# skhu101/TDNN-F_NAS

Hardware: AMD Instinct MI355X
Metric: LF-MMI training frames/sec per node (SWBD 7q TDNN-F) (higher is better)
Workload: dtype f32

## Files before the change

tdnn-f_nas_amd/csrc/abi_tdnn.hip:

```cpp
#include <dlfcn.h>
#include <stdlib.h>
#include <string.h>

#include <string>

#include "common.h"
#include "gemm_f32.h"
#include "planes_gemm.h"

namespace tdnnf {

static thread_local std::string g_last_error;

void set_error(const char *fmt, ...) {
  char buf[1024];
  va_list ap;
  va_start(ap, fmt);
  vsnprintf(buf, sizeof(buf), fmt, ap);
  va_end(ap);
  g_last_error = buf;
}
int hip_status(hipError_t e, const char *what) {
  set_error("HIP error %d (%s) in %s", (int)e, hipGetErrorString(e), what);
  return TDNNF_EHIP;
}

Options &options() {
  static Options o;
  return o;
}

namespace {
typedef int (*roctx_push_t)(const char *);
typedef int (*roctx_pop_t)();
roctx_push_t g_roctx_push = nullptr;
roctx_pop_t g_roctx_pop = nullptr;
bool roctx_ready() {
  static const bool ok = [] {
    const char *e = getenv("TDNNF_ROCTX");
    if (e && atoi(e) == 0) return false;
    for (const char *lib : {"librocprofiler-sdk-roctx.so", "librocprofiler-sdk-roctx.so.1", "libroctx64.so", "libroctx64.so.4"}) {
      void *h = dlopen(lib, RTLD_NOW | RTLD_GLOBAL);
      if (!h) continue;
      g_roctx_push = (roctx_push_t)dlsym(h, "roctxRangePushA");
      g_roctx_pop = (roctx_pop_t)dlsym(h, "roctxRangePop");
      if (g_roctx_push && g_roctx_pop) return true;
    }
    return false;
  }();
  return ok;
}
}
TraceRange::TraceRange(const char *name) : on(roctx_ready()) {
  if (on) g_roctx_push(name);
}
TraceRange::~TraceRange() {
  if (on) g_roctx_pop();
}

static bool tdnn_rows_ok(const tdnnf_tdnn_indexes *ix, int rows_in, int N) {
  if (!ix || ix->num_offsets < 1 || ix->num_offsets > TDNNF_MAX_OFFSETS || ix->row_stride < 1) return false;
  for (int i = 0; i < ix->num_offsets; i++) {
    const long long need = (long long)ix->row_offsets[i] + (long long)ix->row_stride * N - (ix->row_stride - 1);
    if (ix->row_offsets[i] < 0 || (N > 0 && rows_in < need)) return false;
  }
  return true;
}

}

using namespace tdnnf;

extern "C" {

const char *tdnnf_last_error(void) { return g_last_error.c_str(); }
int tdnnf_abi_version(void) { return 1; }

static int *option_slot(const char *name) {
  Options &o = options();
  if (!name) return nullptr;
  const struct { const char *n; int *p; } table[] = {{"ng_grouped", &o.ng_grouped}, {"ng_fuse", &o.ng_fuse}, {"ng_early_in", &o.ng_early_in},
                                                     {"wgrad_stream", &o.wgrad_stream}, {"gemm_ring", &o.gemm_ring}, {"planes", &o.planes}, {"den_split", &o.den_split}, {"phase_events", &o.phase_events}, {"wgrad_lag", &o.wgrad_lag}, {"ng_bk", &o.ng_bk}, {"ng_valu", &o.ng_valu}, {"ng_pform", &o.ng_pform}, {"planes_group", &o.planes_group}, {"xent_behind_den", &o.xent_behind_den}, {"ng_early_fork", &o.ng_early_fork}, {"ng_diag_skip", &o.ng_diag_skip}, {"wgrad_small", &o.wgrad_small}, {"splitk_per_cu", &o.splitk_per_cu}, {"gemm_alt_taps", &o.gemm_alt_taps}, {"reverse_passes", &o.reverse_passes}, {"splitk_partial_round", &o.splitk_partial_round}, {"wgrad_on_caller", &o.wgrad_on_caller}, {"den_mw_test_abort", &o.den_mw_test_abort}, {"planes_check_bound", &o.planes_check_bound}};
  for (auto &e : table)
    if (strcmp(e.n, name) == 0) return e.p;
  return nullptr;
}
int tdnnf_set_option(const char *name, int value) {
  int *p = option_slot(name);
  TDNNF_REQUIRE(p, "set_option: unknown option '%s' (ng_grouped, ng_fuse, ng_early_in, wgrad_stream, gemm_ring, planes, den_split)", name ? name : "(null)");
  *p = value;
  return TDNNF_OK;
}
int tdnnf_get_option(const char *name, int *value) {
  int *p = option_slot(name);
  TDNNF_REQUIRE(p && value, "get_option: unknown option '%s'", name ? name : "(null)");
  *value = *p;
  return TDNNF_OK;
}

}

namespace tdnnf {
int tdnn_propagate_impl(const tdnnf_tdnn_indexes *ix, const tdnnf_mat *in, const float *W, int ldw, int Do, int Di,
                        const float *bias, const float *eff_coef, int init_mode, int relu, tdnnf_mat *out, tdnnf_stream stream,
                        float *colstats, int *colstats_rows) {
  TDNNF_REQUIRE(mat_ok(in) && mat_ok(out) && W, "tdnn_propagate: bad matrices");
  TDNNF_REQUIRE(Do > 0 && Di > 0 && in->cols == Di && out->cols == Do, "tdnn_propagate: dims: in.cols=%d Di=%d out.cols=%d Do=%d",
                in ? in->cols : -1, Di, out ? out->cols : -1, Do);
  TDNNF_REQUIRE(tdnn_rows_ok(ix, in->rows, out->rows), "tdnn_propagate: input has too few rows for the time offsets");
  TDNNF_REQUIRE(ldw >= ix->num_offsets * Di, "tdnn_propagate: ldw < K*Di");
  TDNNF_REQUIRE(init_mode >= 0 && init_mode <= 2 && (init_mode != 1 || bias), "tdnn_propagate: init_mode 1 needs a bias");
  RowsGemmArgs a;
  memset(&a, 0, sizeof(a));
  a.A = in->data;
  a.lda = (long long)in->stride * ix->row_stride;
  a.B = W;
  a.ldb = ldw;
  a.C = out->data;
  a.ldc = out->stride;
  a.M = out->rows;
  a.N = Do;
  a.bias = bias;
  a.coef = eff_coef;
  a.init_mode = init_mode;
  a.relu = relu;
  a.colstats = colstats;
  a.colstats_rows = colstats_rows;
  a.nseg = ix->num_offsets;
  for (int i = 0; i < a.nseg; i++) {
    a.seg[i].a_off = (long long)ix->row_offsets[i] * in->stride;
    a.seg[i].b_off = (long long)i * Di;
    a.seg[i].klen = Di;
    a.seg[i].m_lo = 0;
    a.seg[i].m_hi = out->rows;
  }
  TDNNF_HIP(rows_gemm(a, true, (hipStream_t)stream));
  return TDNNF_OK;
}
}

extern "C" {

int tdnnf_tdnn_propagate(const tdnnf_tdnn_indexes *ix, const tdnnf_mat *in, const float *W, int ldw, int Do, int Di,
                         const float *bias, const float *eff_coef, int init_mode, tdnnf_mat *out, tdnnf_stream stream) {
  return tdnn_propagate_impl(ix, in, W, ldw, Do, Di, bias, eff_coef, init_mode, 0, out, stream);
}

}

namespace tdnnf {
int tdnn_backprop_data_impl(const tdnnf_tdnn_indexes *ix, const tdnnf_mat *out_deriv, const float *W, int ldw, int Do,
                            int Di, const float *eff_coef, int overwrite, const tdnnf_mat *add, float add_scale, int add_lo,
                            tdnnf_mat *in_deriv, tdnnf_stream stream) {
  TDNNF_REQUIRE(mat_ok(in_deriv) && mat_ok(out_deriv) && W, "tdnn_backprop_data: bad matrices");
  TDNNF_REQUIRE(Do > 0 && Di > 0 && in_deriv->cols == Di && out_deriv->cols == Do, "tdnn_backprop_data: bad dims");
  TDNNF_REQUIRE(tdnn_rows_ok(ix, in_deriv->rows, out_deriv->rows), "tdnn_backprop_data: in_deriv has too few rows for the time offsets");
  TDNNF_REQUIRE(ldw >= ix->num_offsets * Di, "tdnn_backprop_data: ldw < K*Di");
  const int rho = ix->row_stride, N = out_deriv->rows, K = ix->num_offsets;
  if (N == 0) return TDNNF_OK;
  for (int cls = 0; cls < rho; cls++) {
    RowsGemmArgs a;
    memset(&a, 0, sizeof(a));
    float cf_dummy = 0;
    (void)cf_dummy;
    int nseg = 0, u_max = 0;
// ... 171 lines not shown
```

tdnn-f_nas_amd/csrc/chain.hip:

```cpp
#include <math.h>
#include <string.h>

#include <algorithm>

#include <vector>

#include "common.h"
#include "gemm_f32.h"

struct tdnnf_den_graph {
  int H, A, P;
  struct Sell {
    int nrows, nslices;
    int *base;
    unsigned *row;
    uint2 *arc;
    uint4 *arc4;
    long long entries;
    int mw_max_arcs[9];
  } by_dst, by_src, by_pdf;
  float *init;
  float init_sum;
};

// ... 519 lines not shown
      }
    }
    const float sum = block_sum(local, red, kDenThreads / 64);
    if (gi == 0 && tid == 0) sums[t] = sum;
    if (DIR == 0) {
      for (int h = tid; h < H; h += kDenThreads) {
        const float a = cur[h] + leaky * sum * g.init[h];
        cur[h] = a;
        if (h >= h0 && h < h1) vec[(size_t)t * Hs + h] = a;
      }
    } else {
      const float is = 1.0f / sum;
      for (int h = tid; h < H; h += kDenThreads) {
        const float v = cur[h];
        if (h >= h0 && h < h1) vec[(size_t)t * Hs + h] = v;
        cur[h] = v * is + leaky;
      }
    }
    if (step < T) row_to_x();
    prev_sum = sum;
    __syncthreads();
  }
  if (DIR == 0) {
    float local = 0.f;
    for (int h = tid; h < H; h += kDenThreads) local += cur[h];
    const float tot = block_sum(local, red, kDenThreads / 64);
    if (gi == 0 && tid == 0) {
      logprob[s] = (double)logf(tot) + logcorr;
      sums[T] = tot;
    }
  }
}

__global__ void den_mw_check_kernel(const unsigned *abort_flag, unsigned *host_fallbacks) {
  if (*abort_flag != 0 && threadIdx.x == 0) __hip_atomic_fetch_add(host_fallbacks, 1u, __ATOMIC_RELAXED, __HIP_MEMORY_SCOPE_SYSTEM);
}

constexpr int kGammaThreads = 512;
__global__ __launch_bounds__(kGammaThreads) void den_gamma_kernel(DenDev g, MatView y, int B, int T, float leaky, const float *alpha_all, const float *b_all,
                                                                  const float *S_all, int Hs, float deriv_weight, MatView deriv) {
  extern __shared__ __attribute__((aligned(16))) float smem[];
  __shared__ float red[kGammaThreads / 64];
  const int t = blockIdx.x, s = blockIdx.y, tid = threadIdx.x;
  const int H = g.H, P = g.P, P4 = (P + 3) & ~3, H4 = (H + 3) & ~3;
  float *x = smem, *ad = smem + P4, *bn = ad + H4;
  const float *alpha = alpha_all + ((size_t)s * (T + 1) + t) * Hs;
  const float *bt = b_all + ((size_t)s * (T + 1) + t) * Hs, *bt1 = bt + Hs;
  const float inv = 1.0f / S_all[(size_t)s * (T + 1) + t + 1];
  const float *yr = y.data + (size_t)(t * B + s) * y.stride;
  for (int p = tid; p < P; p += kGammaThreads) x[p] = exp_limited(yr[p]);
  float local = 0.f;
  for (int h = tid; h < H; h += kGammaThreads) {
    const float a = alpha[h];
    ad[h] = a;
    bn[h] = bt1[h] * inv + leaky;
    local += a * bt[h];
  }
  const float Zd = block_sum(local, red, kGammaThreads / 64);
  const float scale = deriv_weight / Zd;
  float *dr = deriv.data + (size_t)(t * B + s) * deriv.stride;
  constexpr int kRows = 12;
  const int nslot = g.by_pdf.nslices * 64, ln = tid & 63;
  auto term = [&](const uint2 a) { return __uint_as_float(a.y) * ad[a.x & 0xffffu] * bn[a.x >> 16]; };
  for (int s0 = tid; s0 < nslot; s0 += kRows * kGammaThreads) {
    int b0[kRows], w[kRows];
    unsigned row[kRows];
#pragma unroll
    for (int k = 0; k < kRows; k++) {
      const int slot = s0 + k * kGammaThreads;
      b0[k] = 0;
      w[k] = 0;
      row[k] = 0xffffffffu;
      if (slot < nslot) {
        b0[k] = g.by_pdf.base[slot >> 6];
        w[k] = (g.by_pdf.base[(slot >> 6) + 1] - b0[k]) >> 6;
        row[k] = g.by_pdf.row[slot];
      }
    }
#pragma unroll
    for (int k = 0; k < kRows; k++) {
      if (row[k] == 0xffffffffu) continue;
      const float acc = sell_row_sum(g.by_pdf.arc + b0[k] + ln, w[k], term);
      dr[row[k]] = scale * acc * x[row[k]];
    }
  }
}
constexpr int kWideBatch = 8;
constexpr int kWideSlices = 2;

struct WideDims {
  int B, NG, SG;
};

typedef unsigned uv4 __attribute__((ext_vector_type(4)));

__global__ __launch_bounds__(256) void den_wide_prep_kernel(MatView y, WideDims d, int P, float *xT) {
  __shared__ float tile[64][65];
  const int t = blockIdx.z, p0 = blockIdx.x * 64, s0 = blockIdx.y * 64, tx = threadIdx.x & 63, ty = threadIdx.x >> 6;
  for (int i = ty; i < 64; i += 4) {
    const int sq = s0 + i, p = p0 + tx;
    tile[i][tx] = (sq < d.B && p < P) ? exp_limited(y.data[(size_t)(t * d.B + sq) * y.stride + p]) : 0.f;
  }
  __syncthreads();
  for (int i = ty; i < 64; i += 4) {
    const int p = p0 + i, sq = s0 + tx;
    if (p < P && sq < d.NG * d.SG) xT[(((size_t)t * d.NG + sq / d.SG) * P + p) * d.SG + sq % d.SG] = tile[tx][i];
  }
}
__global__ __launch_bounds__(256) void den_wide_unprep_kernel(const float *dT, WideDims d, int P, MatView deriv) {
  __shared__ float tile[64][65];
  const int t = blockIdx.z, p0 = blockIdx.x * 64, s0 = blockIdx.y * 64, tx = threadIdx.x & 63, ty = threadIdx.x >> 6;
  for (int i = ty; i < 64; i += 4) {
    const int p = p0 + i, sq = s0 + tx;
    tile[i][tx] = (p < P && sq < d.B) ? dT[(((size_t)t * d.NG + sq / d.SG) * P + p) * d.SG + sq % d.SG] : 0.f;
  }
  __syncthreads();
  for (int i = ty; i < 64; i += 4) {
    const int sq = s0 + i, p = p0 + tx;
    if (sq < d.B && p < P) deriv.data[(size_t)(t * d.B + sq) * deriv.stride + p] = tile[tx][i];
  }
}

__global__ __launch_bounds__(256) void den_wide_init_kernel(DenDev g, WideDims d, int Hs, bool ones, float *v, float *norm) {
  const long long total = (long long)d.NG * Hs * d.SG;
  for (long long e = blockIdx.x * 256LL + threadIdx.x; e < total; e += gridDim.x * 256LL) {
    const int h = (int)((e / d.SG) % Hs);
    v[e] = h < g.H ? (ones ? 1.0f : g.init[h]) : 0.f;
  }
  for (long long e = blockIdx.x * 256LL + threadIdx.x; e < d.B; e += gridDim.x * 256LL) norm[e] = g.init_sum;
}

template <int SG>
struct WideLane {
  static constexpr int RL = 64 / SG;
  static constexpr int IT = 16 / RL;
  int grp, blk, sl, rl, sq, wave, lane;
  bool on;
  __device__ WideLane(const WideDims &d, int g, int b) {
    lane = threadIdx.x & 63;
    wave = threadIdx.x >> 6;
    grp = g;
    blk = b;
    sl = lane % SG;
    rl = lane / SG;
    sq = grp * SG + sl;
    on = sq < d.B;
  }
};
__device__ __forceinline__ int wide_npad(int nblk) { return (nblk + 3) & ~3; }
template <int SG>
__device__ __forceinline__ float wide_norm(const float *part, int nblk, float *norm_out, float *red, const WideLane<SG> &L) {
  constexpr int NQ = 256 / SG;
  const int q = threadIdx.x / SG, nch = wide_npad(nblk) >> 2;
  const float4 *pp = (const float4 *)(part + ((size_t)L.grp * SG + L.sl) * wide_npad(nblk));
  float v = 0.f;
  for (int c0 = q; c0 < nch; c0 += 8 * NQ) {
    float4 f[8];
#pragma unroll
    for (int u = 0; u < 8; u++) f[u] = c0 + u * NQ < nch ? pp[c0 + u * NQ] : make_float4(0.f, 0.f, 0.f, 0.f);
#pragma unroll
    for (int u = 0; u < 8; u++) v += (f[u].x + f[u].y) + (f[u].z + f[u].w);
  }
  red[q * SG + L.sl] = v;
  __syncthreads();
  float tot = 0.f;
#pragma unroll
// ... 698 lines not shown
    hipStream_t st = nullptr;
    hipEvent_t ef = nullptr, ej = nullptr;
  };
  constexpr int kMaxDev = 64;
  static thread_local Set sets[kMaxDev];
  int dev = 0;
  TDNNF_HIP(hipGetDevice(&dev));
  TDNNF_REQUIRE(dev >= 0 && dev < kMaxDev, "chain: device index %d out of range", dev);
  Set &S = sets[dev];
  if (!S.ef) {
    TDNNF_HIP(hipEventCreateWithFlags(&S.ef, hipEventDisableTiming));
    TDNNF_HIP(hipEventCreateWithFlags(&S.ej, hipEventDisableTiming));
  }
  if (aux && !S.st) TDNNF_HIP(hipStreamCreateWithFlags(&S.st, hipStreamNonBlocking));
  if (aux) *aux = S.st;
  *ev_fork = S.ef;
  *ev_join = S.ej;
  return TDNNF_OK;
}

int chain_den(const tdnnf_den_graph *g, const tdnnf_supervision *sp, const tdnnf_mat *y, float leaky, tdnnf_mat *deriv, void *ws,
              hipStream_t s, bool beside_other_work, hipStream_t caller_aux, hipEvent_t ev_recursions, bool *ev_recorded) {
  if (ev_recorded) *ev_recorded = false;
  const int B = sp->B, T = sp->T;
  ChainBufs b = chain_bufs(g, B, T, ws);
  DenDev gd{g->H, g->P, g->by_dst, g->by_src, g->by_pdf, g->init, g->init_sum};
  MatView yv = view(y), dv = view(deriv);
  ProfHbmRange prof(6, (double)B * T * (24.0 * g->A + 12.0 * g->P), s);
  if (b.p.wide) {
    const int Hs = b.p.Hs, P = g->P;
    const WideDims d{B, b.p.NG, b.p.SG};
    const size_t Bw = (size_t)d.NG * d.SG, frame = Bw * Hs, prow = Bw * b.p.wide_blocks;
    const int nsl = kWideSlices;
    auto blocks = [&](const tdnnf_den_graph::Sell &t) { return (t.nslices + nsl - 1) / nsl; };
    const int nb_dst = blocks(g->by_dst), nb_src = blocks(g->by_src);
    float *alphaT = b.alpha, *asum = b.asum, *S = asum + (size_t)(T + 1) * B, *Zd = S + (size_t)(T + 1) * B;
    float *bT = b.gstate, *part = bT + frame * (T + 1), *part2 = part + 2 * prow, *xT = part2 + 2 * prow;
    const dim3 blk(256), tr((P + 63) / 64, (B + 63) / 64, T), ini(grid_for((long long)frame, 256));
    hipStream_t aux_stream;
    hipEvent_t ev_fork, ev_join;
    {
      int rc = den_aux_stream(&aux_stream, &ev_fork, &ev_join);
      if (rc) return rc;
    }
    hipStream_t aux = aux_stream;
    hipLaunchKernelGGL(den_wide_prep_kernel, tr, blk, 0, s, yv, d, P, xT);
    TDNNF_HIP(hipEventRecord(ev_fork, s));
    TDNNF_HIP(hipStreamWaitEvent(aux, ev_fork, 0));
#define WIDE_LAUNCH(kernel, ...)                                      \
  do {                                                                \
    if (d.SG == 16) hipLaunchKernelGGL(kernel<16>, __VA_ARGS__);      \
    else hipLaunchKernelGGL(kernel<32>, __VA_ARGS__);                 \
  } while (0)
    hipLaunchKernelGGL(den_wide_init_kernel, ini, blk, 0, s, gd, d, Hs, false, alphaT, asum);
    for (int t = 1; t <= T; t++)
      WIDE_LAUNCH(den_wide_fwd_kernel, dim3(nb_dst * d.NG), blk, 0, s, gd, d, t, leaky, xT, alphaT, asum, Hs,
                  t > 1 ? part + (size_t)((t - 1) & 1) * prow : (const float *)nullptr, nb_dst, nsl, part + (size_t)(t & 1) * prow);
    WIDE_LAUNCH(den_wide_sum_kernel, dim3(d.NG), blk, 0, s, part + (size_t)(T & 1) * prow, nb_dst, d, asum + (size_t)T * B);
    hipLaunchKernelGGL(den_wide_total_kernel, dim3((B + 255) / 256), blk, 0, s, gd, B, T, leaky, asum, b.den_lp);
    hipLaunchKernelGGL(den_wide_init_kernel, ini, blk, 0, aux, gd, d, Hs, true, bT + (size_t)T * frame, S + (size_t)T * B);
    for (int t = T - 1; t >= 0; t--)
      WIDE_LAUNCH(den_wide_beta_kernel, dim3(nb_src * d.NG), blk, 0, aux, gd, d, t, leaky, xT, bT + (size_t)(t + 1) * frame, S, Hs, bT + (size_t)t * frame,
                  t < T - 1 ? part2 + (size_t)((t + 1) & 1) * prow : (const float *)nullptr, nb_src, nsl, part2 + (size_t)(t & 1) * prow);
    WIDE_LAUNCH(den_wide_sum_kernel, dim3(d.NG), blk, 0, aux, part2, nb_src, d, S);
    TDNNF_HIP(hipEventRecord(ev_join, aux));
    TDNNF_HIP(hipStreamWaitEvent(s, ev_join, 0));
    WIDE_LAUNCH(den_wide_dot_kernel, dim3(T, d.NG), blk, 0, s, gd, d, leaky, alphaT, asum, Hs, bT, Zd);
    WIDE_LAUNCH(den_wide_gamma_kernel, dim3(g->by_pdf.nslices * d.NG, T), blk, 0, s, gd, d, leaky, xT, alphaT, asum, Hs, bT, S, Zd, -sp->weight);
#undef WIDE_LAUNCH
    hipLaunchKernelGGL(den_wide_unprep_kernel, tr, blk, 0, s, xT, d, P, dv);
    TDNNF_LAUNCH_CHECK();
    return TDNNF_OK;
  }
  if (b.p.split && !beside_other_work) {
    const int P4 = (g->P + 3) & ~3, H4 = (g->H + 3) & ~3;
    const size_t lds_beta = sizeof(float) * (P4 + H4), lds_gamma = sizeof(float) * (P4 + 2 * H4);
    float *b_all = b.gstate, *S_all = b_all + (size_t)B * (T + 1) * b.p.Hs;
    hipEvent_t ev_fork, ev_join;
    hipStream_t aux = caller_aux;
    int rc = den_aux_stream(caller_aux ? nullptr : &aux, &ev_fork, &ev_join);
    if (rc) return rc;
    TDNNF_HIP(hipFuncSetAttribute((const void *)den_forward_kernel<true>, hipFuncAttributeMaxDynamicSharedMemorySize, (int)b.p.lds_fwd));
    TDNNF_HIP(hipFuncSetAttribute((const void *)den_beta_kernel<false>, hipFuncAttributeMaxDynamicSharedMemorySize, (int)lds_beta));
    TDNNF_HIP(hipFuncSetAttribute((const void *)den_gamma_kernel, hipFuncAttributeMaxDynamicSharedMemorySize, (int)lds_gamma));
    TDNNF_HIP(hipEventRecord(ev_fork, s));
    TDNNF_HIP(hipStreamWaitEvent(aux, ev_fork, 0));
    int G = mw_groups(g, B, T);
    MwDev *md = mw_dev();
    if (!md) G = 0;
    if (G > 0 && !md->fallbacks) {
      if (hipHostMalloc((void **)&md->fallbacks, sizeof(unsigned), hipHostMallocMapped) != hipSuccess) {
        (void)hipGetLastError();
        md->fallbacks = nullptr;
        G = 0;
      } else {
        *md->fallbacks = 0;
      }
    }
    if (G > 0 && *(volatile unsigned *)md->fallbacks != 0) {
      fprintf(stderr, "tdnnf: the multi-workgroup denominator recursion timed out (its workgroups were not co-resident); the one-workgroup kernels redid the "
                      "minibatch and are used from here on (this device)\n");
      md->off = true;
      G = 0;
    }
    const size_t stage_b = G > 0 ? 256 * (size_t)((std::max(g->by_dst.nslices, g->by_src.nslices) + G - 1) / G) : 0;
    const size_t lds_f = G > 0 ? sizeof(float) * (P4 + H4) + 8 * (size_t)g->by_dst.mw_max_arcs[G] + stage_b : 0;
    const size_t lds_b = G > 0 ? sizeof(float) * (P4 + H4) + 8 * (size_t)g->by_src.mw_max_arcs[G] + stage_b : 0;
    if (G > 0) {
      TDNNF_HIP(hipFuncSetAttribute((const void *)den_mw_kernel<0>, hipFuncAttributeMaxDynamicSharedMemorySize, (int)lds_f));
      TDNNF_HIP(hipFuncSetAttribute((const void *)den_mw_kernel<1>, hipFuncAttributeMaxDynamicSharedMemorySize, (int)lds_b));
      int occ_f = 0, occ_b = 0;
      if (hipOccupancyMaxActiveBlocksPerMultiprocessor(&occ_f, den_mw_kernel<0>, kDenThreads, lds_f) != hipSuccess ||
          hipOccupancyMaxActiveBlocksPerMultiprocessor(&occ_b, den_mw_kernel<1>, kDenThreads, lds_b) != hipSuccess || occ_f < 1 || occ_b < 1 ||
          md->cus <= 0 || 2 * B * G > md->cus) {
        (void)hipGetLastError();
        G = 0;
      }
    }
    if (G > 0) {
      float *mw = S_all + (size_t)B * (T + 1) + 32;
      MwCtl ctl;
      ctl.NSp = (int)mw_slots(g);
      ctl.ctr = reinterpret_cast<unsigned long long *>((reinterpret_cast<uintptr_t>(mw) + 15) & ~(uintptr_t)15);
      ctl.abort_flag = reinterpret_cast<unsigned *>(ctl.ctr + 2 * B);
      ctl.xf = reinterpret_cast<float *>(ctl.ctr + 2 * B + 2);
      ctl.xb = ctl.xf + (size_t)B * 2 * ctl.NSp;
      TDNNF_HIP(hipMemsetAsync(ctl.ctr, 0, sizeof(unsigned long long) * (2 * B + 2), s));
      if (options().den_mw_test_abort) TDNNF_HIP(hipMemsetAsync(ctl.abort_flag, 1, 1, s));
      TDNNF_HIP(hipEventRecord(ev_fork, s));
      TDNNF_HIP(hipStreamWaitEvent(aux, ev_fork, 0));
      hipLaunchKernelGGL(den_mw_kernel<0>, dim3(B * G), dim3(kDenThreads), lds_f, s, gd, ctl, G, yv, B, T, leaky, b.alpha, b.asum, b.p.Hs, b.den_lp);
      hipLaunchKernelGGL(den_mw_kernel<1>, dim3(B * G), dim3(kDenThreads), lds_b, aux, gd, ctl, G, yv, B, T, leaky, b_all, S_all, b.p.Hs, (double *)nullptr);
      hipLaunchKernelGGL(den_forward_kernel<true>, dim3(B), dim3(kDenThreads), b.p.lds_fwd, s, gd, yv, B, T, leaky, b.alpha, b.asum, b.p.Hs, b.den_lp, b.gstate,
                         (const unsigned *)ctl.abort_flag, 0);
      hipLaunchKernelGGL(den_beta_kernel<false>, dim3(B), dim3(kDenThreads), lds_beta, aux, gd, yv, B, T, leaky, b_all, S_all, b.p.Hs, (const unsigned *)ctl.abort_flag, 0);
      hipLaunchKernelGGL(den_mw_check_kernel, dim3(1), dim3(64), 0, s, (const unsigned *)ctl.abort_flag, md->fallbacks);
    } else {
      const bool fast = g->by_dst.nslices * 64 <= kDenFastSlots * kDenThreads && g->by_src.nslices * 64 <= kDenFastSlots * kDenThreads && g->H <= kDenFastStates * kDenThreads;
      const size_t lf = b.p.lds_fwd + (fast ? sizeof(float) * b.p.Hs : 0), lb = lds_beta + (fast ? sizeof(float) * H4 : 0);
      int res_f = 0, res_b = 0;
      if (md && md->cus > 0 && 2 * B >= md->cus) {
        const size_t budget = 150 * 1024;
        if (lf < budget) res_f = (int)std::min<long long>(g->by_dst.entries, (long long)((budget - lf) / 8)) & ~63;
        if (lb < budget) res_b = (int)std::min<long long>(g->by_src.entries, (long long)((budget - lb) / 8)) & ~63;
      }
      (void)hipGetLastError();
      const size_t lds_f2 = lf + 8 * (size_t)res_f, lds_b2 = lb + 8 * (size_t)res_b;
      if (fast) {
        TDNNF_HIP(hipFuncSetAttribute((const void *)den_forward_kernel<true, true>, hipFuncAttributeMaxDynamicSharedMemorySize, (int)lds_f2));
        TDNNF_HIP(hipFuncSetAttribute((const void *)den_beta_kernel<true>, hipFuncAttributeMaxDynamicSharedMemorySize, (int)lds_b2));
        hipLaunchKernelGGL((den_forward_kernel<true, true>), dim3(B), dim3(kDenThreads), lds_f2, s, gd, yv, B, T, leaky, b.alpha, b.asum, b.p.Hs, b.den_lp, b.gstate,
                           (const unsigned *)nullptr, res_f);
        hipLaunchKernelGGL(den_beta_kernel<true>, dim3(B), dim3(kDenThreads), lds_b2, aux, gd, yv, B, T, leaky, b_all, S_all, b.p.Hs, (const unsigned *)nullptr, res_b);
      } else {
        TDNNF_HIP(hipFuncSetAttribute((const void *)den_forward_kernel<true>, hipFuncAttributeMaxDynamicSharedMemorySize, (int)lds_f2));
        TDNNF_HIP(hipFuncSetAttribute((const void *)den_beta_kernel<false>, hipFuncAttributeMaxDynamicSharedMemorySize, (int)lds_b2));
        hipLaunchKernelGGL(den_forward_kernel<true>, dim3(B), dim3(kDenThreads), lds_f2, s, gd, yv, B, T, leaky, b.alpha, b.asum, b.p.Hs, b.den_lp, b.gstate,
                           (const unsigned *)nullptr, res_f);
        hipLaunchKernelGGL(den_beta_kernel<false>, dim3(B), dim3(kDenThreads), lds_b2, aux, gd, yv, B, T, leaky, b_all, S_all, b.p.Hs, (const unsigned *)nullptr, res_b);
      }
    }
    TDNNF_HIP(hipEventRecord(ev_join, aux));
    TDNNF_HIP(hipStreamWaitEvent(s, ev_join, 0));
    if (ev_recursions) {
      TDNNF_HIP(hipEventRecord(ev_recursions, s));
      if (ev_recorded) *ev_recorded = true;
    }
    hipLaunchKernelGGL(den_gamma_kernel, dim3(T, B), dim3(kGammaThreads), lds_gamma, s, gd, yv, B, T, leaky, b.alpha, b_all, S_all, b.p.Hs, -sp->weight, dv);
  } else if (b.p.lds_state) {
    TDNNF_HIP(hipFuncSetAttribute((const void *)den_backward_kernel<true>, hipFuncAttributeMaxDynamicSharedMemorySize, (int)b.p.lds_bwd));
    if (g->by_dst.nslices * 64 <= kDenFastSlots * kDenThreads && g->H <= kDenFastStates * kDenThreads) {
      const size_t lf = b.p.lds_fwd + sizeof(float) * b.p.Hs;
      TDNNF_HIP(hipFuncSetAttribute((const void *)den_forward_kernel<true, true>, hipFuncAttributeMaxDynamicSharedMemorySize, (int)lf));
      hipLaunchKernelGGL((den_forward_kernel<true, true>), dim3(B), dim3(kDenThreads), lf, s, gd, yv, B, T, leaky, b.alpha, b.asum, b.p.Hs, b.den_lp, b.gstate, (const unsigned *)nullptr, 0);
    } else {
      TDNNF_HIP(hipFuncSetAttribute((const void *)den_forward_kernel<true>, hipFuncAttributeMaxDynamicSharedMemorySize, (int)b.p.lds_fwd));
      hipLaunchKernelGGL(den_forward_kernel<true>, dim3(B), dim3(kDenThreads), b.p.lds_fwd, s, gd, yv, B, T, leaky, b.alpha, b.asum, b.p.Hs, b.den_lp, b.gstate, (const unsigned *)nullptr, 0);
    }
    hipLaunchKernelGGL(den_backward_kernel<true>, dim3(B), dim3(kDenThreads), b.p.lds_bwd, s, gd, yv, B, T, leaky, b.alpha, b.asum, b.p.Hs, -sp->weight, dv, b.gstate);
  } else {
    hipLaunchKernelGGL(den_forward_kernel<false>, dim3(B), dim3(kDenThreads), b.p.lds_fwd, s, gd, yv, B, T, leaky, b.alpha, b.asum, b.p.Hs, b.den_lp, b.gstate, (const unsigned *)nullptr, 0);
    hipLaunchKernelGGL(den_backward_kernel<false>, dim3(B), dim3(kDenThreads), b.p.lds_bwd, s, gd, yv, B, T, leaky, b.alpha, b.asum, b.p.Hs, -sp->weight, dv, b.gstate);
  }
  TDNNF_LAUNCH_CHECK();
  return TDNNF_OK;
}
float chain_supervision_weight(const tdnnf_supervision *sp) { return sp->weight; }
int chain_num_recursion(const tdnnf_supervision *sp, const tdnnf_den_graph *g, const tdnnf_mat *y, void *ws, hipStream_t s) {
  const int B = sp->B, T = sp->T;
  ChainBufs b = chain_bufs(g, B, T, ws);
  const MatView none{nullptr, 0, 0, 0};
  hipLaunchKernelGGL(numerator_kernel, dim3(B), dim3(64), 0, s, sup_dev(sp), view(y), none, b.la, b.lb, b.num_lp, b.xent, none, none, 0.f, 1);
  TDNNF_LAUNCH_CHECK();
  return TDNNF_OK;
}
int chain_num_xent(const tdnnf_den_graph *g, const tdnnf_supervision *sp, const tdnnf_mat *y, const tdnnf_mat *xent_output, float xent_regularize,
                   tdnnf_mat *xent_deriv, void *ws, hipStream_t s, bool xent_deriv_initialised) {
  const int B = sp->B, T = sp->T;
  ChainBufs b = chain_bufs(g, B, T, ws);
  MatView yv = view(y);
  MatView xdv = xent_deriv ? view(xent_deriv) : MatView{nullptr, 0, 0, 0};
  MatView xov = xent_output ? view(xent_output) : MatView{nullptr, 0, 0, 0};
  if (xent_deriv && !xent_deriv_initialised) {
    if (xdv.stride == xdv.cols) TDNNF_HIP(hipMemsetAsync(xdv.data, 0, sizeof(float) * (size_t)xdv.rows * xdv.cols, s));
    else hipLaunchKernelGGL(zero_rows_kernel, dim3(grid_for((long long)xdv.rows * xdv.cols, 256)), dim3(256), 0, s, xdv);
  }
  hipLaunchKernelGGL(numerator_kernel, dim3(B), dim3(64), 0, s, sup_dev(sp), yv, xov, b.la, b.lb, b.num_lp, b.xent, MatView{nullptr, 0, 0, 0},
                     xdv, xent_regularize, 4);
  TDNNF_LAUNCH_CHECK();
  return TDNNF_OK;
}
int chain_num(const tdnnf_den_graph *g, const tdnnf_supervision *sp, const tdnnf_mat *y, const tdnnf_mat *xent_output,
              float xent_regularize, tdnnf_mat *xent_deriv, void *ws, hipStream_t s, bool xent_deriv_initialised) {
  int rc = chain_num_recursion(sp, g, y, ws, s);
  if (rc) return rc;
  return chain_num_xent(g, sp, y, xent_output, xent_regularize, xent_deriv, ws, s, xent_deriv_initialised);
}
int chain_finish(const tdnnf_den_graph *g, const tdnnf_supervision *sp, const tdnnf_mat *y, float l2_regularize, double *results,
                 tdnnf_mat *deriv, tdnnf_mat *xent_deriv, void *ws, hipStream_t s) {
  const int B = sp->B, T = sp->T;
  ChainBufs b = chain_bufs(g, B, T, ws);
  MatView yv = view(y), dv = view(deriv);
  MatView xdv = xent_deriv ? view(xent_deriv) : MatView{nullptr, 0, 0, 0};
  hipLaunchKernelGGL(numerator_kernel, dim3(B), dim3(64), 0, s, sup_dev(sp), yv, MatView{nullptr, 0, 0, 0}, b.la, b.lb, b.num_lp, b.xent, dv,
                     MatView{nullptr, 0, 0, 0}, 0.f, 2);
  if (l2_regularize != 0.f) {
    TDNNF_HIP(hipMemsetAsync(b.l2sum, 0, sizeof(double), s));
    hipLaunchKernelGGL(sumsq_kernel, dim3(grid_for((long long)yv.rows * yv.cols, 256, 1024)), dim3(256), 0, s, yv, b.l2sum);
  }
  hipLaunchKernelGGL(chain_finalize_kernel, dim3(1), dim3(64), 0, s, b.num_lp, b.den_lp, b.xent, l2_regularize != 0.f ? b.l2sum : nullptr,
                     B, T, sp->weight, l2_regularize, results);
  hipLaunchKernelGGL(chain_guard_kernel, dim3(grid_for((long long)dv.rows * dv.cols, 256)), dim3(256), 0, s, results, yv,
                     sp->weight * l2_regularize, dv, xdv);
  TDNNF_LAUNCH_CHECK();
  return TDNNF_OK;
}
}

extern "C" {

int tdnnf_chain_objf_and_deriv(const tdnnf_den_graph *g, const tdnnf_supervision *sp, const tdnnf_mat *y,
                               const tdnnf_mat *xent_output, float leaky, float l2_regularize, float xent_regularize,
                               double *results, tdnnf_mat *deriv, tdnnf_mat *xent_deriv, void *ws, size_t ws_bytes,
                               tdnnf_stream stream) {
  TDNNF_REQUIRE(g && sp && mat_ok(y) && mat_ok(deriv) && results, "chain_objf_and_deriv: bad arguments");
  const int B = sp->B, T = sp->T;
  TDNNF_REQUIRE(y->rows == B * T && y->cols == g->P && same_dim(y, deriv), "chain_objf_and_deriv: nnet_output must be (B*T) x num_pdfs, t-major");
  TDNNF_REQUIRE(!xent_deriv || (mat_ok(xent_deriv) && same_dim(y, xent_deriv)), "chain_objf_and_deriv: bad xent_deriv");
  TDNNF_REQUIRE(!xent_output || (mat_ok(xent_output) && same_dim(y, xent_output)), "chain_objf_and_deriv: bad xent_output");
  TDNNF_REQUIRE(sp->num_states <= B * 4 * (T + 1), "chain_objf_and_deriv: supervision has more than 4*(T+1) states per sequence on average");
  TDNNF_REQUIRE(ws && ws_bytes >= tdnnf_chain_workspace_bytes(g, B, T), "chain_objf_and_deriv: workspace too small");
// ... 9 lines not shown
```

tdnn-f_nas_amd/csrc/common.h:

```cpp
#pragma once
#include <hip/hip_runtime.h>
#include <stdarg.h>
#include <stdio.h>

#include "tdnnf_hip.h"

namespace tdnnf {

struct MatView {
  float *data;
  int rows, cols, stride;
};
inline MatView view(const tdnnf_mat *m) { return MatView{m->data, m->rows, m->cols, m->stride}; }

void set_error(const char *fmt, ...);
int hip_status(hipError_t e, const char *what);

inline bool mat_ok(const tdnnf_mat *m) {
  return m && m->rows >= 0 && m->cols >= 0 && m->stride >= m->cols && (m->data || m->rows * m->cols == 0);
}
inline bool same_dim(const tdnnf_mat *a, const tdnnf_mat *b) { return a->rows == b->rows && a->cols == b->cols; }

inline bool vec4_ok(const MatView &m) {
  return (reinterpret_cast<uintptr_t>(m.data) & 15) == 0 && m.stride % 4 == 0 && m.cols % 4 == 0;
}

#define TDNNF_REQUIRE(cond, ...)            \
  do {                                      \
    if (!(cond)) {                          \
      ::tdnnf::set_error(__VA_ARGS__);      \
      return TDNNF_EINVAL;                  \
    }                                       \
  } while (0)

#define TDNNF_HIP(expr)                                         \
  do {                                                          \
    hipError_t e__ = (expr);                                    \
    if (e__ != hipSuccess) return ::tdnnf::hip_status(e__, #expr); \
  } while (0)

#define TDNNF_LAUNCH_CHECK(name) TDNNF_HIP(hipGetLastError())

struct Options {
  int ng_grouped = 1;
  int ng_fuse = 1;
  int ng_early_in = 1;
  int wgrad_stream = -1;
  int gemm_ring = 1;
  int planes = 1;
  int den_mw_test_abort = 0;
  int planes_group = 1;
  int planes_check_bound = 0;
  int wgrad_lag = 3;
  int wgrad_on_caller = 0;
  int splitk_partial_round = 1;
  int reverse_passes = 0;
  int gemm_alt_taps = 1;
  int splitk_per_cu = 2;
  int wgrad_small = 0;
  int ng_bk = 0;
  int ng_early_fork = 1;
  int xent_behind_den = -1;
  int ng_pform = 1;
  int ng_valu = 0;
  int ng_diag_skip = 0;
  int phase_events = 0;
  int den_split = -1;
};
Options &options();

struct TraceRange {
  explicit TraceRange(const char *name);
  ~TraceRange();
  bool on;
};

__host__ __device__ inline float floor_keep_nan(float x, float f) { return x < f ? f : x; }

inline int grid_for(long long work, int block, int cap = 2048) {
  long long g = (work + block - 1) / block;
  if (g > cap) g = cap;
  if (g < 1) g = 1;
  return (int)g;
}

inline unsigned long long tdnnf_decision(unsigned long long step, unsigned long long k) {
  unsigned long long z = step * 0x9E3779B97F4A7C15ULL + k * 0xBF58476D1CE4E5B9ULL + 0x94D049BB133111EBULL;
  z = (z ^ (z >> 30)) * 0xBF58476D1CE4E5B9ULL;
  z = (z ^ (z >> 27)) * 0x94D049BB133111EBULL;
  return (z ^ (z >> 31)) >> 8;
}

constexpr int kFinCols = 8, kFinLanes = 32, kFinThreads = kFinCols * kFinLanes;
inline unsigned finalize_grid(int D) { return (unsigned)((D + kFinCols - 1) / kFinCols); }
#ifdef __HIPCC__
template <int NQ, class Acc>
__device__ __forceinline__ void finalize_sums(const float *partial, int chunks, long long qstride_rows, int D, int nq, Acc (&q)[NQ], Acc *red) {
  const int tc = threadIdx.x & (kFinCols - 1), lane = threadIdx.x / kFinCols, d = blockIdx.x * kFinCols + tc;
#pragma unroll
  for (int k = 0; k < NQ; k++) q[k] = 0;
  if (d < D) {
    const float *p = partial + d;
    const long long qs = qstride_rows * D;
    int c = lane;
    for (; c + 3 * kFinLanes < chunks; c += 4 * kFinLanes) {
      float v[NQ][4];
#pragma unroll
      for (int k = 0; k < NQ; k++) {
        if (k < nq) {
          const float *pk = p + (long long)k * qs;
          v[k][0] = pk[(long long)c * D]; v[k][1] = pk[(long long)(c + kFinLanes) * D];
          v[k][2] = pk[(long long)(c + 2 * kFinLanes) * D]; v[k][3] = pk[(long long)(c + 3 * kFinLanes) * D];
        }
      }
#pragma unroll
      for (int k = 0; k < NQ; k++) {
        if (k < nq) { q[k] += v[k][0]; q[k] += v[k][1]; q[k] += v[k][2]; q[k] += v[k][3]; }
      }
    }
    for (; c < chunks; c += kFinLanes) {
      float v[NQ];
#pragma unroll
      for (int k = 0; k < NQ; k++)
        if (k < nq) v[k] = p[(long long)k * qs + (long long)c * D];
#pragma unroll
      for (int k = 0; k < NQ; k++)
        if (k < nq) q[k] += v[k];
    }
  }
#pragma unroll
  for (int k = 0; k < NQ; k++) red[(k * kFinLanes + lane) * (kFinCols + 1) + tc] = q[k];
  __syncthreads();
  if (lane == 0) {
#pragma unroll
    for (int k = 0; k < NQ; k++) {
      Acc s = 0;
      for (int l = 0; l < kFinLanes; l++) s += red[(k * kFinLanes + l) * (kFinCols + 1) + tc];
      q[k] = s;
    }
  }
}
#endif

struct BnSync {
  int (*fn)(void *ctx, double *buf, long long count, tdnnf_stream stream);
  void *ctx;
  double *buf;
  int world;
};
BnSync *bn_sync_current();
// ... 52 lines not shown
```

Baseline: 1.599 million.

## Process two frames per workgroup in denominator gamma kernel to reuse arc reads

Adds a den_gamma2 kernel in which each workgroup handles two consecutive frames. Each sparse arc entry loaded from the by_pdf SELL structure is applied to both frames' alpha/beta values held in LDS, so arc metadata traffic per frame is halved. It uses twice the threads and twice the LDS per block. The kernel is on by default whenever that fits in the LDS budget, and an option restores the one-frame kernel. The cost is higher LDS use per block, which may reduce occupancy, plus more register pressure from the dual accumulators.

After: 1.630 million (median of 6 runs). +1.9%, better.

```diff
diff --git a/tdnn-f_nas_amd/csrc/abi_tdnn.hip b/tdnn-f_nas_amd/csrc/abi_tdnn.hip
--- a/tdnn-f_nas_amd/csrc/abi_tdnn.hip
+++ b/tdnn-f_nas_amd/csrc/abi_tdnn.hip
@@ -80,7 +80,7 @@
   Options &o = options();
   if (!name) return nullptr;
   const struct { const char *n; int *p; } table[] = {{"ng_grouped", &o.ng_grouped}, {"ng_fuse", &o.ng_fuse}, {"ng_early_in", &o.ng_early_in},
-                                                     {"wgrad_stream", &o.wgrad_stream}, {"gemm_ring", &o.gemm_ring}, {"planes", &o.planes}, {"den_split", &o.den_split}, {"phase_events", &o.phase_events}, {"wgrad_lag", &o.wgrad_lag}, {"ng_bk", &o.ng_bk}, {"ng_valu", &o.ng_valu}, {"ng_pform", &o.ng_pform}, {"planes_group", &o.planes_group}, {"xent_behind_den", &o.xent_behind_den}, {"ng_early_fork", &o.ng_early_fork}, {"ng_diag_skip", &o.ng_diag_skip}, {"wgrad_small", &o.wgrad_small}, {"splitk_per_cu", &o.splitk_per_cu}, {"gemm_alt_taps", &o.gemm_alt_taps}, {"reverse_passes", &o.reverse_passes}, {"splitk_partial_round", &o.splitk_partial_round}, {"wgrad_on_caller", &o.wgrad_on_caller}, {"den_mw_test_abort", &o.den_mw_test_abort}, {"planes_check_bound", &o.planes_check_bound}};
+                                                     {"wgrad_stream", &o.wgrad_stream}, {"gemm_ring", &o.gemm_ring}, {"planes", &o.planes}, {"den_split", &o.den_split}, {"phase_events", &o.phase_events}, {"wgrad_lag", &o.wgrad_lag}, {"ng_bk", &o.ng_bk}, {"ng_valu", &o.ng_valu}, {"ng_pform", &o.ng_pform}, {"planes_group", &o.planes_group}, {"xent_behind_den", &o.xent_behind_den}, {"ng_early_fork", &o.ng_early_fork}, {"ng_diag_skip", &o.ng_diag_skip}, {"wgrad_small", &o.wgrad_small}, {"splitk_per_cu", &o.splitk_per_cu}, {"gemm_alt_taps", &o.gemm_alt_taps}, {"reverse_passes", &o.reverse_passes}, {"splitk_partial_round", &o.splitk_partial_round}, {"wgrad_on_caller", &o.wgrad_on_caller}, {"den_mw_test_abort", &o.den_mw_test_abort}, {"planes_check_bound", &o.planes_check_bound}, {"den_gamma_pairs", &o.den_gamma_pairs}};
   for (auto &e : table)
     if (strcmp(e.n, name) == 0) return e.p;
   return nullptr;
diff --git a/tdnn-f_nas_amd/csrc/chain.hip b/tdnn-f_nas_amd/csrc/chain.hip
--- a/tdnn-f_nas_amd/csrc/chain.hip
+++ b/tdnn-f_nas_amd/csrc/chain.hip
@@ -625,6 +625,147 @@
       if (row[k] == 0xffffffffu) continue;
       const float acc = sell_row_sum(g.by_pdf.arc + b0[k] + ln, w[k], term);
       dr[row[k]] = scale * acc * x[row[k]];
+    }
+  }
+}
+
+template <int N, class Fa, class Fb>
+__device__ __forceinline__ void sell_row_sums(const uint2 *ap, int w, float (&acc)[N], Fa pa, Fb pb) {
+#pragma clang fp contract(off)
+#pragma unroll
+  for (int n = 0; n < N; n++) acc[n] = 0.f;
+  int j = 0;
+  for (; j + 8 <= w; j += 8) {
+    uint2 a[8];
+#pragma unroll
+    for (int u = 0; u < 8; u++) a[u] = ap[(j + u) * 64];
+#pragma unroll
+    for (int u = 0; u < 8; u++)
+#pragma unroll
+      for (int n = 0; n < N; n++) acc[n] += pa(a[u], n) * pb(a[u], n);
+  }
+  if (j + 4 <= w) {
+    uint2 a[4];
+#pragma unroll
+    for (int u = 0; u < 4; u++) a[u] = ap[(j + u) * 64];
+#pragma unroll
+    for (int u = 0; u < 4; u++)
+#pragma unroll
+      for (int n = 0; n < N; n++) acc[n] += pa(a[u], n) * pb(a[u], n);
+    j += 4;
+  }
+  if (j < w) {
+    uint2 a[3];
+#pragma unroll
+    for (int u = 0; u < 3; u++) a[u] = ap[min(j + u, w - 1) * 64];
+#pragma unroll
+    for (int n = 0; n < N; n++) acc[n] = __builtin_fmaf(pa(a[0], n), pb(a[0], n), acc[n]);
+#pragma unroll
+    for (int u = 1; u < 3; u++)
+#pragma unroll
+      for (int n = 0; n < N; n++) acc[n] += (j + u < w) ? pa(a[u], n) * pb(a[u], n) : 0.f;
+  }
+}
+
+constexpr int kGamma2Threads = 2 * kGammaThreads;
+constexpr size_t kLdsBytes = 160 * 1024;
+__global__ __launch_bounds__(kGamma2Threads) void den_gamma2_kernel(DenDev g, MatView y, int B, int T, float leaky, const float *alpha_all, const float *b_all,
+                                                                    const float *S_all, int Hs, float deriv_weight, MatView deriv) {
+  extern __shared__ __attribute__((aligned(16))) float smem[];
+  __shared__ float red[kGamma2Threads / 64];
+  const int t0 = 2 * blockIdx.x, s = blockIdx.y, tid = threadIdx.x;
+  const int H = g.H, P = g.P, P4 = (P + 3) & ~3, H4 = (H + 3) & ~3, L = 2 * H4 + P4;
+  const int nf = min(2, T - t0);
+  {
+    const int f = tid / kGammaThreads, ht = tid % kGammaThreads, t = min(t0 + f, T - 1);
+    float *ad = smem + f * L, *bn = ad + H4;
+    const float *alpha = alpha_all + ((size_t)s * (T + 1) + t) * Hs;
+    const float *bt = b_all + ((size_t)s * (T + 1) + t) * Hs, *bt1 = bt + Hs;
+    const float inv = 1.0f / S_all[(size_t)s * (T + 1) + t + 1];
+    constexpr int kBatch = 8;
+    float local = 0.f;
+    for (int h0 = ht; h0 < H; h0 += kBatch * kGammaThreads) {
+      float av[kBatch], bv[kBatch], b1v[kBatch];
+#pragma unroll
+      for (int i = 0; i < kBatch; i++) {
+        const int h = h0 + i * kGammaThreads;
+        av[i] = h < H ? alpha[h] : 0.f;
+        bv[i] = h < H ? bt[h] : 0.f;
+        b1v[i] = h < H ? bt1[h] : 0.f;
+      }
+#pragma unroll
+      for (int i = 0; i < kBatch; i++) {
+        const int h = h0 + i * kGammaThreads;
+        if (h < H) {
+          ad[h] = av[i];
+          bn[h] = __builtin_fmaf(b1v[i], inv, leaky);
+        }
+        local = __builtin_fmaf(av[i], bv[i], local);
+      }
+    }
+    for (int o = 32; o > 0; o >>= 1) local += __shfl_xor(local, o, 64);
+    if ((tid & 63) == 0) red[tid >> 6] = local;
+  }
+  __syncthreads();
+  float scale[2];
+#pragma unroll
+  for (int f = 0; f < 2; f++) {
+    float Zd = 0.f;
+    for (int w = 0; w < kGammaThreads / 64; w++) Zd += red[f * (kGammaThreads / 64) + w];
+    scale[f] = deriv_weight / Zd;
+  }
+  constexpr int kRows = 8;
+  const int nslot = g.by_pdf.nslices * 64, ln = tid & 63;
+  auto pa = [&](const uint2 a, int f) {
+#pragma clang fp contract(off)
+    return __uint_as_float(a.y) * smem[f * L + (a.x & 0xffffu)];
+  };
+  auto pb = [&](const uint2 a, int f) { return smem[f * L + H4 + (a.x >> 16)]; };
+  for (int s0 = tid; s0 < nslot; s0 += kRows * kGamma2Threads) {
+    int b0[kRows], w[kRows];
+    unsigned row[kRows];
+#pragma unroll
+    for (int k = 0; k < kRows; k++) {
+      const int slot = s0 + k * kGamma2Threads;
+      b0[k] = 0;
+      w[k] = 0;
+      row[k] = 0xffffffffu;
+      if (slot < nslot) {
+        b0[k] = g.by_pdf.base[slot >> 6];
+        w[k] = (g.by_pdf.base[(slot >> 6) + 1] - b0[k]) >> 6;
+        row[k] = g.by_pdf.row[slot];
+      }
+    }
+#pragma unroll
+    for (int k = 0; k < kRows; k++) {
+      if (row[k] == 0xffffffffu) continue;
+      float acc[2];
+      sell_row_sums<2>(g.by_pdf.arc + b0[k] + ln, w[k], acc, pa, pb);
+#pragma unroll
+      for (int f = 0; f < 2; f++) smem[f * L + 2 * H4 + row[k]] = scale[f] * acc[f];
+    }
+  }
+  __syncthreads();
+  constexpr int kOut = 6;
+  for (int p0 = tid; p0 < P; p0 += kOut * kGamma2Threads) {
+    float yv[2][kOut];
+#pragma unroll
+    for (int f = 0; f < 2; f++)
+#pragma unroll
+      for (int i = 0; i < kOut; i++) {
+        const int p = p0 + i * kGamma2Threads;
+        yv[f][i] = f < nf && p < P ? y.data[(size_t)((t0 + f) * B + s) * y.stride + p] : 0.f;
+      }
+#pragma unroll
+    for (int f = 0; f < 2; f++) {
+      if (f >= nf) break;
+      const float *o = smem + f * L + 2 * H4;
+      float *dr = deriv.data + (size_t)((t0 + f) * B + s) * deriv.stride;
+#pragma unroll
+      for (int i = 0; i < kOut; i++) {
+        const int p = p0 + i * kGamma2Threads;
+        if (p < P) dr[p] = o[p] * exp_limited(yv[f][i]);
+      }
     }
   }
 }
@@ -1489,7 +1630,6 @@
     if (rc) return rc;
     TDNNF_HIP(hipFuncSetAttribute((const void *)den_forward_kernel<true>, hipFuncAttributeMaxDynamicSharedMemorySize, (int)b.p.lds_fwd));
     TDNNF_HIP(hipFuncSetAttribute((const void *)den_beta_kernel<false>, hipFuncAttributeMaxDynamicSharedMemorySize, (int)lds_beta));
-    TDNNF_HIP(hipFuncSetAttribute((const void *)den_gamma_kernel, hipFuncAttributeMaxDynamicSharedMemorySize, (int)lds_gamma));
     TDNNF_HIP(hipEventRecord(ev_fork, s));
     TDNNF_HIP(hipStreamWaitEvent(aux, ev_fork, 0));
     int G = mw_groups(g, B, T);
@@ -1573,7 +1713,13 @@
       TDNNF_HIP(hipEventRecord(ev_recursions, s));
       if (ev_recorded) *ev_recorded = true;
     }
-    hipLaunchKernelGGL(den_gamma_kernel, dim3(T, B), dim3(kGammaThreads), lds_gamma, s, gd, yv, B, T, leaky, b.alpha, b_all, S_all, b.p.Hs, -sp->weight, dv);
+    if (options().den_gamma_pairs != 1 && 2 * lds_gamma + sizeof(float) * kGamma2Threads / 64 <= kLdsBytes) {
+      TDNNF_HIP(hipFuncSetAttribute((const void *)den_gamma2_kernel, hipFuncAttributeMaxDynamicSharedMemorySize, (int)(2 * lds_gamma)));
+      hipLaunchKernelGGL(den_gamma2_kernel, dim3((T + 1) / 2, B), dim3(kGamma2Threads), 2 * lds_gamma, s, gd, yv, B, T, leaky, b.alpha, b_all, S_all, b.p.Hs, -sp->weight, dv);
+    } else {
+      TDNNF_HIP(hipFuncSetAttribute((const void *)den_gamma_kernel, hipFuncAttributeMaxDynamicSharedMemorySize, (int)lds_gamma));
+      hipLaunchKernelGGL(den_gamma_kernel, dim3(T, B), dim3(kGammaThreads), lds_gamma, s, gd, yv, B, T, leaky, b.alpha, b_all, S_all, b.p.Hs, -sp->weight, dv);
+    }
   } else if (b.p.lds_state) {
     TDNNF_HIP(hipFuncSetAttribute((const void *)den_backward_kernel<true>, hipFuncAttributeMaxDynamicSharedMemorySize, (int)b.p.lds_bwd));
     if (g->by_dst.nslices * 64 <= kDenFastSlots * kDenThreads && g->H <= kDenFastStates * kDenThreads) {
diff --git a/tdnn-f_nas_amd/csrc/common.h b/tdnn-f_nas_amd/csrc/common.h
--- a/tdnn-f_nas_amd/csrc/common.h
+++ b/tdnn-f_nas_amd/csrc/common.h
@@ -66,6 +66,7 @@
   int ng_diag_skip = 0;
   int phase_events = 0;
   int den_split = -1;
+  int den_gamma_pairs = 0;
 };
 Options &options();
 
```
